# chrischoy/DeepGlobalRegistration

Measured on NVIDIA H100. Metric: scan_pairs_per_sec, higher is better.
Workload: dtype f32

## Files before the change

### deepglobalregistration_b200/_abi.py

```python
import ctypes as C
import math
import os
import re

import numpy as np
import torch

from .build import INCLUDE

_HERE = os.path.dirname(os.path.abspath(__file__))
LIB_PATH = os.path.join(_HERE, 'libdgr_b200.so')
HEADER = os.path.join(INCLUDE, 'dgr_b200.h')


class DgrError(RuntimeError):
  pass


_SCALARS = {'int32_t': C.c_int32, 'int64_t': C.c_int64, 'uint64_t': C.c_uint64, 'float': C.c_float,
            'double': C.c_double}


def _ctype(decl, c_type, ret=False):
  words = c_type.replace('*', ' * ').split()
# ... 252 lines not shown
  call('dgr_hash_find', ptr(coords), coords.shape[0], coords.shape[1], ptr(spec), ptr(table.keys),
       ptr(table.vals), table.cap, ptr(rows), stream())
  return rows


def gather_rows_i32(src, idx, n):
  out = torch.empty(n, src.shape[1], dtype=torch.int32, device=src.device)
  call('dgr_gather_rows_i32', ptr(src), ptr(idx), n, src.shape[1], ptr(out), stream())
  return out


def coarse_maps(fine, spec, strides):
  _chk(fine, torch.int32, 'fine')
  n, ncols = fine.shape
  L, nmx, dev = len(strides), max(n, 1), fine.device
  cap = table_cap(n)
  keys = torch.empty(L, cap, dtype=torch.int64, device=dev)
  vals = torch.empty(L, cap, dtype=torch.int32, device=dev)
  coords = torch.empty(L, nmx, ncols, dtype=torch.int32, device=dev)
  n_out = torch.empty(L, dtype=torch.int32, device=dev)
  slot = scratch('cm_slot', L * nmx, torch.int32, dev)
  scan = scratch('cm_scan', L * lib().dgr_scan_ws_elems(nmx), torch.int32, dev)
  call('dgr_coarse_maps', ptr(fine), n, None, ncols, ptr(spec), L, (C.c_int32 * L)(*strides), ptr(keys), ptr(vals),
       cap, ptr(coords), ptr(n_out), ptr(slot), ptr(scan), stream())
  return coords, [HashTable.wrap(keys[l], vals[l], cap) for l in range(L)], n_out


class KernelMap:
  __slots__ = ('K', 'n_in', 'n_out', 'nbr', 'in_idx', 'out_idx', 'kofs', 'kofs_host', 'n_pairs',
               'tile_k', 'tile_start', 'n_tiles', '_paired')

  def paired_tiles(self):
    if getattr(self, '_paired', None) is None:
      counts = self.kofs_host[1:] - self.kofs_host[:-1]
      per_k = (counts + TILE_ROWS - 1) // TILE_ROWS
      n = int(((per_k + 1) // 2 * 2).sum())
      dev = self.kofs.device
      tk = torch.empty(max(n, 1), dtype=torch.int32, device=dev)
      ts = torch.empty(max(n, 1), dtype=torch.int32, device=dev)
      call('dgr_kernel_map_tiles', ptr(self.kofs), self.K, TILE_ROWS, n, 1, ptr(tk), ptr(ts), stream())
      self._paired = (tk, ts, n)
    return self._paired

  def transposed(self):
    t = KernelMap()
    for k in self.__slots__:
      setattr(t, k, getattr(self, k, None))
    t.in_idx, t.out_idx = self.out_idx, self.in_idx
    t.n_in, t.n_out = self.n_out, self.n_in
    t.nbr = None
    return t


def kernel_map(out_coords, spec, in_table, n_in, offsets, keep_table=False):
  global D2H_BYTES
  _chk(out_coords, torch.int32, 'out_coords')
  _chk(offsets, torch.int32, 'offsets')
  dev = out_coords.device
  n_out, ncols = out_coords.shape
  K = offsets.shape[0]
  nmx = max(n_out, 1)
  bits = scratch('km_bits', K * lib().dgr_kmap_mask_words(nmx), torch.int32, dev)
  cnt = scratch('km_cnt', lib().dgr_kmap_cnt_elems(K, nmx), torch.int32, dev)
  kofs = torch.empty(K + 2, dtype=torch.int32, device=dev)
  meta = scratch('km_meta', 5, torch.int32, dev)
  bloom, n_words = None, 0
  if K > 27:
    n_words = lib().dgr_bloom2_words(n_in)
    bloom = scratch('km_bloom', n_words, torch.int32, dev)
    call('dgr_bloom2_build', ptr(in_table.keys), in_table.cap, ptr(bloom), n_words, stream())
  table = (ptr(in_table.keys), ptr(in_table.vals), in_table.cap)
  call('dgr_kmap_probe', ptr(out_coords), n_out, None, ncols, ptr(spec), *table, ptr(bloom), n_words, ptr(offsets), K,
       ptr(bits), ptr(cnt), ptr(kofs), ptr(meta), stream())
  km = KernelMap()
  km.nbr = None
  if keep_table:
    km.nbr = torch.empty(K, nmx, dtype=torch.int32, device=dev)
    call('dgr_kmap_dense', ptr(out_coords), n_out, None, ncols, ptr(spec), *table, ptr(bloom), n_words, ptr(offsets),
         K, ptr(km.nbr), nmx, None, stream())
  kofs_all = kofs.cpu().numpy()
  D2H_BYTES += kofs_all.nbytes
  if kofs_all[K + 1] != 0:
    raise DgrError('coordinate extent does not fit a 63-bit packed key')
  kofs_host = kofs_all[:K + 1]
  P = int(kofs_host[K])
  counts = kofs_host[1:] - kofs_host[:-1]
  n_tiles = int(((counts + TILE_ROWS - 1) // TILE_ROWS).sum())
  km.K, km.n_in, km.n_out = K, n_in, n_out
  km.in_idx = torch.empty(max(P, 1), dtype=torch.int32, device=dev)
  km.out_idx = torch.empty(max(P, 1), dtype=torch.int32, device=dev)
  km.tile_k = torch.empty(max(n_tiles, 1), dtype=torch.int32, device=dev)
  km.tile_start = torch.empty(max(n_tiles, 1), dtype=torch.int32, device=dev)
  if P > 0:
    call('dgr_kmap_fill', ptr(bits), ptr(cnt), K, n_out, ptr(out_coords), ncols, ptr(spec), *table, ptr(offsets),
         ptr(km.in_idx), ptr(km.out_idx), stream())
    call('dgr_kernel_map_tiles', ptr(kofs), K, TILE_ROWS, n_tiles, 0, ptr(km.tile_k), ptr(km.tile_start), stream())
  km.kofs, km.kofs_host, km.n_pairs, km.n_tiles = kofs, kofs_host, P, n_tiles
  km._paired = None
  return km


def spconv_fwd(feat, weight, km, out, relu_in=False):
  _chk(feat, torch.float32, 'feat'); _chk(weight, torch.float32, 'weight'); _chk(out, torch.float32, 'out')
  cin, cout = feat.shape[1], out.shape[1]
  assert weight.numel() == km.K * cin * cout, (weight.shape, km.K, cin, cout)
  assert feat.shape[0] == km.n_in and out.shape[0] == km.n_out, (feat.shape, out.shape, km.n_in, km.n_out)
  _conv_profiled('spconv_fwd_kernel', km, cin, cout, lambda: call(
      'dgr_spconv_fwd', ptr(feat), cin, ptr(weight), cout, ptr(km.in_idx), ptr(km.out_idx), ptr(km.kofs),
      ptr(km.tile_k), ptr(km.tile_start), km.n_tiles, TILE_ROWS, int(relu_in), ptr(out), stream()))
  return out


def spconv_wgrad(feat, grad_out, km):
  _chk(feat, torch.float32, 'feat'); _chk(grad_out, torch.float32, 'grad_out')
  cin, cout = feat.shape[1], grad_out.shape[1]
  dw = torch.empty(km.K, cin, cout, dtype=torch.float32, device=feat.device)
  call('dgr_spconv_wgrad', ptr(feat), cin, ptr(grad_out), cout, ptr(km.in_idx), ptr(km.out_idx), ptr(km.kofs), km.K,
       ptr(dw), stream())
  return dw


def tc_supported(cin, cout):
  return bool(lib().dgr_spconv_tc_supported(int(cin), int(cout)))


# ... 656 lines not shown
```

### deepglobalregistration_b200/csrc/coordplan.cu

```cuda
#include "common.cuh"

namespace {

constexpr int kThreads = 256;
constexpr int kCntWords = 256;
constexpr int kProbeThreads = 512;

template <typename T0, typename T1>
__global__ void compact_voxels_kernel(const int32_t* __restrict__ raw, const int32_t* __restrict__ sel,
                                      const int32_t* __restrict__ n_unique, int64_t n_raw0,
                                      const T0* __restrict__ xyz0, const T1* __restrict__ xyz1, double cell,
                                      int32_t* __restrict__ coords, float* __restrict__ xyz,
                                      int32_t* __restrict__ counts) {
  const int n = n_unique[0];
  if (blockIdx.x == 0 && threadIdx.x == 0) {
    int lo = 0, hi = n;
    while (lo < hi) {
      const int mid = (lo + hi) >> 1;
      if (sel[mid] < n_raw0) lo = mid + 1; else hi = mid;
    }
    counts[0] = n;
    counts[1] = lo;
    counts[2] = n - lo;
    counts[3] = n_unique[1];
  }
  for (int64_t i = (int64_t)blockIdx.x * blockDim.x + threadIdx.x; i < n; i += (int64_t)gridDim.x * blockDim.x) {
    const int64_t r = sel[i];
    const int4 k = reinterpret_cast<const int4*>(raw)[r];
    reinterpret_cast<int4*>(coords)[i] = k;
    double x, y, z;
    if (r < n_raw0) {
      x = (double)xyz0[3 * r]; y = (double)xyz0[3 * r + 1]; z = (double)xyz0[3 * r + 2];
    } else {
      const int64_t q = r - n_raw0;
      x = (double)xyz1[3 * q]; y = (double)xyz1[3 * q + 1]; z = (double)xyz1[3 * q + 2];
    }
    xyz[3 * i] = dgr_float32_in_cell(x, k.y, cell);
    xyz[3 * i + 1] = dgr_float32_in_cell(y, k.z, cell);
    xyz[3 * i + 2] = dgr_float32_in_cell(z, k.w, cell);
  }
}

__device__ __forceinline__ uint32_t bloom_mix(uint64_t key) {
  uint32_t h = (uint32_t)key ^ ((uint32_t)(key >> 32) * 0x9E3779B1u);
  h ^= h >> 16;
  h *= 0x85EBCA6Bu;
  h ^= h >> 13;
  h *= 0xC2B2AE35u;
  h ^= h >> 16;
  return h;
}
__device__ __forceinline__ uint32_t bloom_bits(uint32_t h) { return (1u << ((h >> 20) & 31)) | (1u << ((h >> 26) & 31)); }

__global__ void bloom2_build_kernel(const uint64_t* __restrict__ keys, int64_t cap, uint32_t* words,
                                    uint32_t word_mask) {
  int64_t i = (int64_t)blockIdx.x * blockDim.x + threadIdx.x;
  if (i >= cap) return;
  const uint64_t k = keys[i];
  if (k == DGR_EMPTY_KEY) return;
  const uint32_t h = bloom_mix(k);
  atomicOr(words + (h & word_mask), bloom_bits(h));
}

template <bool kBloom, bool kDense>
__global__ void __launch_bounds__(kProbeThreads, 2)
kmap_probe_kernel(const int32_t* __restrict__ out_coords, const int32_t* __restrict__ n_out_dev, int64_t n_out_max,
                  int ncols, const dgr_keyspec_t* __restrict__ spec_p, const uint64_t* __restrict__ keys,
                  const int32_t* __restrict__ vals, uint64_t mask, const uint32_t* __restrict__ bloom,
                  uint32_t n_bloom_words, const int32_t* __restrict__ offsets, int K, int k_per_block,
                  uint32_t* __restrict__ bits, int W, int32_t* block_cnt, int bpk, int32_t* __restrict__ nbr,
                  int64_t nbr_stride, int32_t* hit_count) {
  extern __shared__ __align__(16) unsigned char smem_raw[];
  constexpr int kWarps = kProbeThreads / 32;
  long long* delta = reinterpret_cast<long long*>(smem_raw);
  uint32_t* mtile = reinterpret_cast<uint32_t*>(smem_raw + (size_t)k_per_block * 8);
  uint16_t* queue = reinterpret_cast<uint16_t*>(mtile + (size_t)kWarps * k_per_block);
  uint32_t* bloom_s = reinterpret_cast<uint32_t*>(queue + kWarps * 64);
  const int n_out = dgr_dev_count(n_out_dev, n_out_max);
  const int k0 = blockIdx.y * k_per_block;
  const int kn = min(k_per_block, K - k0);
  const int lane = threadIdx.x & 31, warp = threadIdx.x >> 5;
  if ((int64_t)blockIdx.x * kProbeThreads >= n_out) {
    if (!kDense) {
      const int w = blockIdx.x * kWarps + warp;
      if (lane == 0 && w < W)
        for (int kk = 0; kk < kn; ++kk) bits[(int64_t)(k0 + kk) * W + w] = 0u;
    }
    return;
  }
  const dgr_keyspec_t s = *spec_p;
  for (int kk = threadIdx.x; kk < kn; kk += blockDim.x) {
    long long d = 0;
    const int32_t* o = offsets + (int64_t)(k0 + kk) * (ncols - 1);
    for (int a = 0; a < ncols - 1; ++a) d += (long long)o[a] * (1ll << s.shift[a + 1]);
    delta[kk] = d;
  }
  if (!kDense)
    for (int e = threadIdx.x; e < kWarps * k_per_block; e += blockDim.x) mtile[e] = 0u;
  if (kBloom)
    for (uint32_t i = threadIdx.x; i < n_bloom_words; i += blockDim.x) bloom_s[i] = bloom[i];
  __syncthreads();
  const int64_t j = (int64_t)blockIdx.x * kProbeThreads + threadIdx.x;
  const bool live = j < n_out;
  const uint64_t key = live ? dgr_pack_key(out_coords + j * ncols, s) : 0;
  const uint32_t key_lo = (uint32_t)key, key_hi = (uint32_t)(key >> 32);
  const int64_t row0 = j - lane;
  const uint32_t wm = n_bloom_words - 1;
  uint16_t* q = queue + warp * 64;
  uint32_t* mt = mtile + warp * k_per_block;
  int qn = 0;

  auto drain = [&](int count) {
    __syncwarp();
    const uint32_t e = lane < count ? q[lane] : 0u;
    const int src = e & 31, kq = e >> 5;
    const uint32_t lo = __shfl_sync(0xffffffffu, key_lo, src), hi = __shfl_sync(0xffffffffu, key_hi, src);
    if (lane < count) {
      const uint64_t qq = (((uint64_t)hi << 32) | lo) + (uint64_t)delta[kq];
      const int32_t i = dgr_hash_lookup(keys, vals, mask, qq);
      if (kDense) {
        nbr[(int64_t)(k0 + kq) * nbr_stride + row0 + src] = i;
        if (hit_count != nullptr) {
          const uint32_t act = __activemask();
          const uint32_t hits = __ballot_sync(act, i >= 0);
          if (lane == (__ffs(act) - 1) && hits) atomicAdd(hit_count, __popc(hits));
        }
      } else if (i >= 0) {
        atomicOr(mt + kq, 1u << src);
      }
    }
    __syncwarp();
    const uint32_t rest = (lane + 32 < qn) ? q[lane + 32] : 0u;
    __syncwarp();
    if (lane + 32 < qn) q[lane] = (uint16_t)rest;
    qn = qn > 32 ? qn - 32 : 0;
    __syncwarp();
  };

  if (!kBloom && !kDense) {
    const int w = (int)(j >> 5);
    const int cnt_col = w / kCntWords;
    for (int kk = 0; kk < kn; kk += 4) {
      bool found[4];
#pragma unroll
      for (int u = 0; u < 4; ++u)
        found[u] = live && kk + u < kn && dgr_hash_lookup(keys, vals, mask, key + (uint64_t)delta[min(kk + u, kn - 1)]) >= 0;
#pragma unroll
      for (int u = 0; u < 4; ++u) {
        if (kk + u >= kn) break;
        const uint32_t m = __ballot_sync(0xffffffffu, found[u]);
        if (lane == 0 && w < W) {
          bits[(int64_t)(k0 + kk + u) * W + w] = m;
          if (m) atomicAdd(block_cnt + (int64_t)(k0 + kk + u) * bpk + cnt_col, __popc(m));
        }
      }
    }
    return;
  }
  for (int kk = 0; kk < kn; ++kk) {
    bool maybe = live;
    if (kBloom && live) {
      const uint32_t h = bloom_mix(key + (uint64_t)delta[kk]);
      const uint32_t b = bloom_bits(h);
      maybe = (bloom_s[h & wm] & b) == b;
    }
    if (kDense && live && !maybe) nbr[(int64_t)(k0 + kk) * nbr_stride + j] = -1;
    const uint32_t cand = __ballot_sync(0xffffffffu, maybe);
    if (cand) {
      if (maybe) q[qn + __popc(cand & ((1u << lane) - 1u))] = (uint16_t)((kk << 5) | lane);
      qn += __popc(cand);
      if (qn >= 32) drain(32);
    }
  }
  if (qn > 0) drain(qn);
  if (!kDense) {
    __syncwarp();
    const int w = (int)(j >> 5);
    if (w < W) {
      const int cnt_col = w / kCntWords;
      for (int kk = lane; kk < kn; kk += 32) {
        const uint32_t m = mt[kk];
        bits[(int64_t)(k0 + kk) * W + w] = m;
        if (m) atomicAdd(block_cnt + (int64_t)(k0 + kk) * bpk + cnt_col, __popc(m));
      }
    }
  }
}

__global__ void kmap_scan_kernel(int32_t* cnt, int K, int bpk, int tile_rows, int32_t* kofs,
                                 int32_t* meta, const dgr_keyspec_t* spec) {
  const int64_t nb = (int64_t)K * bpk;
  const int total = dgr_block_scan_inplace(cnt, nb);
  if (threadIdx.x == 0) cnt[nb] = total;
  __syncthreads();
  __shared__ int red[3][32];
  int tiles = 0, ptiles = 0, nonempty = 0;
  for (int k = threadIdx.x; k <= K; k += blockDim.x) {
    const int lo = cnt[(int64_t)k * bpk];
    kofs[k] = lo;
    if (k < K) {
      const int hi = (k + 1 < K) ? cnt[(int64_t)(k + 1) * bpk] : total;
      const int t = (hi - lo + tile_rows - 1) / tile_rows;
      tiles += t;
      ptiles += (t + 1) & ~1;
      nonempty += (hi > lo);
    }
  }
#pragma unroll
  for (int d = 16; d > 0; d >>= 1) {
    tiles += __shfl_xor_sync(0xffffffffu, tiles, d);
    ptiles += __shfl_xor_sync(0xffffffffu, ptiles, d);
    nonempty += __shfl_xor_sync(0xffffffffu, nonempty, d);
  }
  if ((threadIdx.x & 31) == 0) {
    red[0][threadIdx.x >> 5] = tiles;
    red[1][threadIdx.x >> 5] = ptiles;
    red[2][threadIdx.x >> 5] = nonempty;
  }
  __syncthreads();
  if (threadIdx.x == 0) {
    int a = 0, b = 0, c = 0;
    for (int w = 0; w < (int)(blockDim.x >> 5); ++w) { a += red[0][w]; b += red[1][w]; c += red[2][w]; }
    const int ovf = spec != nullptr ? spec->overflow : 0;
    kofs[K + 1] = ovf;
    meta[0] = total; meta[1] = a; meta[2] = b; meta[3] = c; meta[4] = ovf;
  }
}

__global__ void __launch_bounds__(kThreads)
kmap_fill_kernel(const uint32_t* __restrict__ bits, int W, int bpk, const int32_t* __restrict__ block_ofs,
                 const int32_t* __restrict__ out_coords, int ncols, const dgr_keyspec_t* __restrict__ spec_p,
                 const uint64_t* __restrict__ keys, const int32_t* __restrict__ vals, uint64_t mask,
                 const int32_t* __restrict__ offsets, int32_t* __restrict__ in_idx, int32_t* __restrict__ out_idx) {
  __shared__ uint32_t s_mask[kThreads];
  __shared__ int s_base[kThreads];
  const int kappa = blockIdx.y;
  const int64_t e = (int64_t)kappa * bpk + blockIdx.x;
  const int base = block_ofs[e];
  if (block_ofs[e + 1] == base) return;
// ... 57 lines not shown
  const int64_t n_max = n_raw0 + n_raw1;
  unsigned blocks = dgr_blocks(n_max > 0 ? n_max : 1, kThreads);
  if (blocks > 1184) blocks = 1184;
#define DGR_CV(T0, T1)                                                                                         \
  compact_voxels_kernel<T0, T1><<<blocks, kThreads, 0, st>>>(raw_coords, sel, n_unique, n_raw0, (const T0*)xyz0, \
                                                             (const T1*)xyz1, cell, coords, xyz, counts)
  if (is_f64_0 && is_f64_1) DGR_CV(double, double);
  else if (is_f64_0) DGR_CV(double, float);
  else if (is_f64_1) DGR_CV(float, double);
  else DGR_CV(float, float);
#undef DGR_CV
  dgr_note_launches(1);
  DGR_LAUNCH_CHECK();
  return DGR_OK;
}

int32_t dgr_bloom2_build(const uint64_t* keys, int64_t cap, uint32_t* words, int64_t n_words, void* stream) {
  DGR_ARG_CHECK(cap > 0 && (cap & (cap - 1)) == 0, "capacity must be a power of two");
  DGR_ARG_CHECK(n_words >= 32 && (n_words & (n_words - 1)) == 0, "n_words must be a power of two");
  cudaStream_t st = (cudaStream_t)stream;
  DGR_CUDA_CHECK(cudaMemsetAsync(words, 0, (size_t)n_words * 4, st));
  bloom2_build_kernel<<<dgr_blocks(cap, kThreads), kThreads, 0, st>>>(keys, cap, words, (uint32_t)n_words - 1);
  dgr_note_launches(1);
  DGR_LAUNCH_CHECK();
  return DGR_OK;
}

int64_t dgr_bloom2_words(int64_t n_max) {
  int64_t words = 1;
  while (words < (n_max * 10 + 31) / 32) words <<= 1;
  return words < 1024 ? 1024 : (words > 16384 ? 16384 : words);
}

int64_t dgr_kmap_mask_words(int64_t n_out_max) {
  const int64_t w = (n_out_max + 31) / 32;
  return w < 1 ? 1 : w;
}
int64_t dgr_kmap_cnt_elems(int32_t K, int64_t n_out_max) {
  const int64_t W = dgr_kmap_mask_words(n_out_max);
  return (int64_t)K * ((W + kCntWords - 1) / kCntWords) + 2;
}

static size_t probe_smem_bytes(int k_per_block, int64_t n_bloom_words) {
  return (size_t)k_per_block * 8 + (size_t)(kProbeThreads / 32) * k_per_block * 4 + (size_t)(kProbeThreads / 32) * 64 * 2 +
         (size_t)n_bloom_words * 4;
}
static int probe_k_per_block(int K, unsigned row_blocks) {
  int k_per_block = K;
  while (k_per_block > 16 && (int64_t)row_blocks * ((K + k_per_block - 1) / k_per_block) < 528) k_per_block = (k_per_block + 1) / 2;
  if (k_per_block > 96) k_per_block = 96;
  return (k_per_block + 3) & ~3;
}

int32_t dgr_kmap_probe(const int32_t* out_coords, int64_t n_out_max, const int32_t* n_out_dev, int32_t ncols,
                       const dgr_keyspec_t* spec, const uint64_t* in_keys, const int32_t* in_vals, int64_t in_cap,
                       const uint32_t* bloom_words, int64_t n_bloom_words, const int32_t* offsets, int32_t K,
                       uint32_t* bits, int32_t* block_cnt, int32_t* kofs, int32_t* meta, void* stream) {
  DGR_ARG_CHECK(in_cap > 0 && (in_cap & (in_cap - 1)) == 0, "capacity must be a power of two");
  DGR_ARG_CHECK(K >= 1 && K <= 65535, "K out of range");
  DGR_ARG_CHECK(bloom_words == nullptr || (n_bloom_words >= 32 && (n_bloom_words & (n_bloom_words - 1)) == 0 &&
                                           n_bloom_words <= 32768),
                "bloom: power of two, 32..32768 words");
  cudaStream_t st = (cudaStream_t)stream;
  const int64_t nmx = n_out_max > 0 ? n_out_max : 1;
  const int W = (int)dgr_kmap_mask_words(nmx);
  const int bpk = (W + kCntWords - 1) / kCntWords;
  DGR_CUDA_CHECK(cudaMemsetAsync(block_cnt, 0, (size_t)dgr_kmap_cnt_elems(K, nmx) * sizeof(int32_t), st));
  const unsigned row_blocks = dgr_blocks(nmx, kProbeThreads);
  const int k_per_block = probe_k_per_block(K, row_blocks);
  const dim3 grid(row_blocks, (K + k_per_block - 1) / k_per_block);
  if (bloom_words != nullptr) {
    const size_t smem = probe_smem_bytes(k_per_block, n_bloom_words);
    DGR_ENSURE_SMEM((kmap_probe_kernel<true, false>), smem);
    kmap_probe_kernel<true, false><<<grid, kProbeThreads, smem, st>>>(
        out_coords, n_out_dev, n_out_max, ncols, spec, in_keys, in_vals, (uint64_t)in_cap - 1, bloom_words,
        (uint32_t)n_bloom_words, offsets, K, k_per_block, bits, W, block_cnt, bpk, nullptr, 0, nullptr);
  } else {
    const size_t smem = probe_smem_bytes(k_per_block, 0);
    kmap_probe_kernel<false, false><<<grid, kProbeThreads, smem, st>>>(
        out_coords, n_out_dev, n_out_max, ncols, spec, in_keys, in_vals, (uint64_t)in_cap - 1, nullptr, 1u, offsets, K,
        k_per_block, bits, W, block_cnt, bpk, nullptr, 0, nullptr);
  }
  kmap_scan_kernel<<<1, 1024, 0, st>>>(block_cnt, K, bpk, 128, kofs, meta, spec);
  dgr_note_launches(2);
  DGR_LAUNCH_CHECK();
  return DGR_OK;
}

int32_t dgr_kmap_fill(const uint32_t* bits, const int32_t* block_cnt, int32_t K, int64_t n_out_max,
                      const int32_t* out_coords, int32_t ncols, const dgr_keyspec_t* spec,
                      const uint64_t* in_keys, const int32_t* in_vals, int64_t in_cap, const int32_t* offsets,
                      int32_t* in_idx, int32_t* out_idx, void* stream) {
  const int64_t nmx = n_out_max > 0 ? n_out_max : 1;
  const int W = (int)dgr_kmap_mask_words(nmx);
  const int bpk = (W + kCntWords - 1) / kCntWords;
  kmap_fill_kernel<<<dim3(bpk, K), kThreads, 0, (cudaStream_t)stream>>>(bits, W, bpk, block_cnt, out_coords, ncols,
                                                                            spec, in_keys, in_vals, (uint64_t)in_cap - 1,
                                                                            offsets, in_idx, out_idx);
  dgr_note_launches(1);
  DGR_LAUNCH_CHECK();
  return DGR_OK;
}

int32_t dgr_kmap_dense(const int32_t* out_coords, int64_t n_out_max, const int32_t* n_out_dev, int32_t ncols,
                       const dgr_keyspec_t* spec, const uint64_t* in_keys, const int32_t* in_vals, int64_t in_cap,
                       const uint32_t* bloom_words, int64_t n_bloom_words, const int32_t* offsets, int32_t K,
                       int32_t* nbr, int64_t nbr_stride, int32_t* hit_count, void* stream) {
  DGR_ARG_CHECK(in_cap > 0 && (in_cap & (in_cap - 1)) == 0, "capacity must be a power of two");
  DGR_ARG_CHECK(nbr_stride >= n_out_max, "row stride below the row bound");
  if (hit_count != nullptr) DGR_CUDA_CHECK(cudaMemsetAsync(hit_count, 0, sizeof(int32_t), (cudaStream_t)stream));
  DGR_ARG_CHECK(bloom_words == nullptr || (n_bloom_words >= 32 && (n_bloom_words & (n_bloom_words - 1)) == 0 &&
                                           n_bloom_words <= 32768),
                "bloom: power of two, 32..32768 words");
  if (n_out_max == 0) return DGR_OK;
  cudaStream_t st = (cudaStream_t)stream;
  const unsigned row_blocks = dgr_blocks(n_out_max, kProbeThreads);
  const int k_per_block = probe_k_per_block(K, row_blocks);
  const dim3 grid(row_blocks, (K + k_per_block - 1) / k_per_block);
  if (bloom_words != nullptr) {
    const size_t smem = probe_smem_bytes(k_per_block, n_bloom_words);
    DGR_ENSURE_SMEM((kmap_probe_kernel<true, true>), smem);
    kmap_probe_kernel<true, true><<<grid, kProbeThreads, smem, st>>>(
        out_coords, n_out_dev, n_out_max, ncols, spec, in_keys, in_vals, (uint64_t)in_cap - 1, bloom_words,
        (uint32_t)n_bloom_words, offsets, K, k_per_block, nullptr, 0, nullptr, 0, nbr, nbr_stride, hit_count);
  } else {
    const size_t smem = probe_smem_bytes(k_per_block, 0);
    kmap_probe_kernel<false, true><<<grid, kProbeThreads, smem, st>>>(
        out_coords, n_out_dev, n_out_max, ncols, spec, in_keys, in_vals, (uint64_t)in_cap - 1, nullptr, 1u, offsets, K,
        k_per_block, nullptr, 0, nullptr, 0, nbr, nbr_stride, hit_count);
  }
  dgr_note_launches(1);
  DGR_LAUNCH_CHECK();
  return DGR_OK;
}

int32_t dgr_kernel_map_tiles(const int32_t* kofs, int32_t K, int32_t tile_rows, int32_t n_tiles, int32_t pair,
                             int32_t* tile_k, int32_t* tile_start, void* stream) {
  DGR_ARG_CHECK(tile_rows >= 1, "tile_rows must be positive");
  if (n_tiles == 0) return DGR_OK;
  tiles_kernel<<<1, 1024, (K + 1) * sizeof(int), (cudaStream_t)stream>>>(kofs, K, tile_rows, n_tiles, pair, tile_k,
                                                                        tile_start);
  dgr_note_launches(1);
  DGR_LAUNCH_CHECK();
  return DGR_OK;
}

}
```

### deepglobalregistration_b200/csrc/exec.cu

```cuda
#include <math.h>
#include <stdlib.h>
#include <string.h>

#include <map>
#include <tuple>
#include <vector>

#include <nvtx3/nvToolsExt.h>

#include "common.cuh"

namespace {

constexpr int kTileRows = 128;
constexpr int kMetaInts = 256;
constexpr int kMetaNetBase = 8;
constexpr int kMetaPerMap = 5;
constexpr int kKeyMargin = 32;

bool tc_f16_enabled();
int tc_f16_min_cout();

__global__ void fill_f32_kernel(float* p, int64_t n, float v) {
  int64_t i = (int64_t)blockIdx.x * blockDim.x + threadIdx.x;
// ... 293 lines not shown
    L.n_max = n_max;
    L.n_dev = n_out_dev + (l - 1);
    L.keys = keys + (int64_t)(l - 1) * cap;
    L.vals = vals + (int64_t)(l - 1) * cap;
    L.cap = cap;
  }
  const bool use_bloom = p.D > 3;
  if (use_bloom || net->conv1_ks > 3) {
    const int64_t words = dgr_bloom2_words(n_max);
    for (int l = 0; l < (use_bloom ? 4 : 1); ++l) {
      DGR_TRY(aalloc(c, words, &p.lv[l].bloom));
      p.lv[l].n_bloom = words;
      DGR_TRY(dgr_bloom2_build(p.lv[l].keys, p.lv[l].cap, p.lv[l].bloom, words, st));
    }
  }
  p.n_maps = 0;
  auto add_map = [&](int lin, int lout, int ksize, bool dense) {
    KMap& m = p.maps[p.n_maps];
    m = KMap();
    m.lin = lin; m.lout = lout; m.ksize = ksize; m.dense = dense;
    m.K = 1;
    for (int a = 0; a < p.D; ++a) m.K *= ksize;
    return p.n_maps++;
  };
  for (int l = 0; l < 4; ++l) p.map_same[l] = add_map(l, l, 3, false);
  for (int l = 0; l < 3; ++l) p.map_down[l] = add_map(l, l + 1, 3, false);
  if (net->conv1_ks == 3) {
    p.map_conv1 = p.map_same[0];
  } else {
    const bool bits_only = conv1_table_kernel(net) && p.input_ones && net->in_ch == 1;
    p.map_conv1 = add_map(0, 0, net->conv1_ks, conv1_table_kernel(net) && !bits_only);
    p.maps[p.map_conv1].bits_only = bits_only;
  }
  for (int i = 0; i < p.n_maps; ++i) {
    KMap& m = p.maps[i];
    const Level& Lin = p.lv[m.lin];
    const Level& Lout = p.lv[m.lout];
    DGR_TRY(get_offsets(c, m.ksize, p.D, 1 << m.lin, &m.offsets));
    m.meta = c->meta_dev + p.meta_base + 4 + kMetaPerMap * i;
    if (m.dense) {
      m.nbr_stride = nmx;
      DGR_TRY(aalloc(c, (int64_t)m.K * nmx, &m.nbr));
      const bool bloom = Lin.bloom != nullptr && m.K > 27;
      DGR_CUDA_CHECK(cudaMemsetAsync(m.meta, 0, kMetaPerMap * sizeof(int32_t), (cudaStream_t)st));
      DGR_TRY(dgr_kmap_dense(Lout.coords, Lout.n_max, Lout.n_dev, ncols, p.spec, Lin.keys, Lin.vals, Lin.cap,
                             bloom ? Lin.bloom : nullptr, bloom ? Lin.n_bloom : 0, m.offsets, m.K, m.nbr, m.nbr_stride,
                             m.meta, st));
      continue;
    }
    m.W = dgr_kmap_mask_words(nmx);
    DGR_TRY(aalloc(c, (int64_t)m.K * m.W, &m.bits));
    DGR_TRY(aalloc(c, dgr_kmap_cnt_elems(m.K, nmx), &m.cnt));
    DGR_TRY(aalloc(c, m.K + 2, &m.kofs));
    const bool bloom = Lin.bloom != nullptr && m.K > 27;
    DGR_TRY(dgr_kmap_probe(Lout.coords, Lout.n_max, Lout.n_dev, ncols, p.spec, Lin.keys, Lin.vals, Lin.cap,
                           bloom ? Lin.bloom : nullptr, bloom ? Lin.n_bloom : 0, m.offsets, m.K, m.bits, m.cnt, m.kofs,
                           m.meta, st));
  }
  return DGR_OK;
}

int32_t plan_finish(dgr_ctx* c, Plan& p) {
  void* st = c->stream;
  const int32_t* mh = c->meta_host + p.meta_base;
  for (int l = 1; l < 4; ++l) p.lv[l].n = mh[l];
  for (int i = 0; i < p.n_maps; ++i) {
    KMap& m = p.maps[i];
    const int32_t* mm = mh + 4 + kMetaPerMap * i;
    if (m.dense || m.bits_only) {
      m.P = mm[0];
      m.nonempty = m.dense ? m.K : mm[3];
      continue;
    }
    m.P = mm[0]; m.n_tiles = mm[1]; m.nonempty = mm[3];
    if (mm[4] != 0) {
      dgr_set_error("coordinate extent does not fit a 63-bit packed key");
      return DGR_ERR_ARG;
    }
    const Level& Lin = p.lv[m.lin];
    const Level& Lout = p.lv[m.lout];
    DGR_TRY(aalloc(c, m.P, &m.in_idx));
    DGR_TRY(aalloc(c, m.P, &m.out_idx));
    DGR_TRY(aalloc(c, m.n_tiles, &m.tile_k));
    DGR_TRY(aalloc(c, m.n_tiles, &m.tile_start));
    if (m.P > 0) {
      DGR_TRY(dgr_kmap_fill(m.bits, m.cnt, m.K, Lout.n_max > 0 ? Lout.n_max : 1, Lout.coords, p.ncols, p.spec, Lin.keys,
                            Lin.vals, Lin.cap, m.offsets, m.in_idx, m.out_idx, st));
      DGR_TRY(dgr_kernel_map_tiles(m.kofs, m.K, kTileRows, m.n_tiles, 0, m.tile_k, m.tile_start, st));
    }
  }
  return DGR_OK;
}

struct LayerExec {
  const Conv* conv;
  const KMap* map;
  bool transposed;
  int n_in, n_out;
  bool table;
  bool bits;
};

bool tc_f16_enabled() {
  static const bool v = [] {
    const char* e = getenv("DGR_TC_F16");
    return e ? atoi(e) != 0 : true;
  }();
  return v;
}
int tc_f16_min_cout() {
// ... 600 lines not shown
```

### deepglobalregistration_b200/me/coords.py

```python
import numpy as np
import torch

from .. import _abi
from .._abi import KEY_MARGIN


class CoordinateMapKey:
  __slots__ = ('stride', 'tag')

  def __init__(self, stride, tag=''):
    self.stride, self.tag = int(stride), tag

  def get_tensor_stride(self):
    return self.stride

  def __eq__(self, o):
    return isinstance(o, CoordinateMapKey) and (self.stride, self.tag) == (o.stride, o.tag)

  def __hash__(self):
    return hash((self.stride, self.tag))

  def __repr__(self):
    return f'CoordinateMapKey(stride={self.stride})'

# ... 30 lines not shown
      spec = _abi.keyspec_build(_abi.coords_minmax(coords), coords.shape[1], KEY_MARGIN)
      table, _, _, cnt = _abi.unique_first(coords, spec)
      n_unique = _abi.read_count(cnt)
      if n_unique != coords.shape[0]:
        raise ValueError(f'{coords.shape[0] - n_unique} duplicate coordinates: the DGR hot path feeds '
                         'unique coordinates (sparse_quantize output) and relies on row order')
    coords = coords.detach()
    self.device = coords.device
    self.D = coords.shape[1] - 1
    self.spec = spec
    self._maps = {1: _Map(coords, table, coords.shape[0])}
    self._kmaps = {}
    self._offsets = {}

  @staticmethod
  def _check_spec(spec):
    if int(spec[1].item()) != 0:
      raise _abi.DgrError('coordinate extent does not fit a 63-bit packed key')

  def origin_key(self):
    return CoordinateMapKey(1)

  def num_rows(self, key):
    return self._map(key.stride).n

  def coordinates(self, key):
    return self._map(key.stride).coords

  def _map(self, stride):
    if stride not in self._maps:
      assert stride % 2 == 0 and stride > 1, f'no coordinate map at stride {stride}'
      coords, tables, n_out = _abi.coarse_maps(self._maps[1].coords, self.spec, [stride])
      n, overflow = torch.cat([n_out, self.spec[1:2]]).cpu().tolist()
      _abi.D2H_BYTES += 8
      if overflow:
        raise _abi.DgrError('coordinate extent does not fit a 63-bit packed key')
      self._maps[stride] = _Map(coords[0, :n], tables[0], n)
    return self._maps[stride]

  def _offs(self, kernel_size, stride):
    k = (kernel_size, self.D, stride, self.device)
    if k not in _OFFSET_CACHE:
      _OFFSET_CACHE[k] = kernel_offsets(kernel_size, self.D, stride, self.device)
    return _OFFSET_CACHE[k]

  def kernel_map(self, in_key, conv_stride, kernel_size):
    s_in = in_key.stride
    s_out = s_in * conv_stride
    ck = (s_in, s_out, kernel_size)
    if ck not in self._kmaps:
      m_in, m_out = self._map(s_in), self._map(s_out)
      keep = self.D == 3 and conv_stride == 1 and kernel_size > 3
      self._kmaps[ck] = _abi.kernel_map(m_out.coords, self.spec, m_in.table, m_in.n,
                                        self._offs(kernel_size, s_in), keep_table=keep)
    return CoordinateMapKey(s_out), self._kmaps[ck]

  def transpose_kernel_map(self, in_key, conv_stride, kernel_size):
    s_in = in_key.stride
    assert s_in % conv_stride == 0, 'transposed convolution below tensor stride 1'
    s_out = s_in // conv_stride
    if conv_stride == 1:
      return self.kernel_map(in_key, 1, kernel_size)
    ck = (s_out, s_in, kernel_size)
    if ck not in self._kmaps:
      raise NotImplementedError('transposed convolution without a matching strided convolution '
                                '(generating new coordinates) is not on the DGR hot path')
    tk = ('T',) + ck
    if tk not in self._kmaps:
      self._kmaps[tk] = self._kmaps[ck].transposed()
    return CoordinateMapKey(s_out), self._kmaps[tk]
```

### include/dgr_b200.h

```cpp
#ifndef DGR_B200_H_
#define DGR_B200_H_

#include <stdint.h>

#ifdef __cplusplus
extern "C" {
#endif

#define DGR_OK 0
#define DGR_ERR_CUDA (-1)
#define DGR_ERR_ARG (-2)
#define DGR_ERR_DEVICE (-3)

#define DGR_MAX_COLS 8

typedef struct dgr_keyspec {
  int32_t ncols;
  int32_t overflow;
  int32_t lo[DGR_MAX_COLS];
  int32_t shift[DGR_MAX_COLS];
  int32_t bits[DGR_MAX_COLS];
} dgr_keyspec_t;

int32_t dgr_version(void);
// ... 211 lines not shown
                      int32_t* base_log, double* result, void* stream);

#define DGR_POINTNET_PARAMS 154368
#define DGR_POINTNET_PACKED_BYTES 1185792
int32_t dgr_pointnet_pack(const double* params, void* packed, void* stream);
int32_t dgr_pointnet_forward(const float* points, int64_t n, const double* centre, const double* poses, int32_t n_poses,
                             const void* packed, float* features, void* stream);
int32_t dgr_pointnetlk_ws_elems(int64_t n_src, int64_t n_tgt, int32_t max_iter, int64_t* n_elems);
int32_t dgr_pointnetlk(const float* src, int64_t n_src, const float* tgt, int64_t n_tgt, const void* packed,
                       double delta, int32_t max_iter, double xtol, uint64_t* ws, double* jac_out, double* log,
                       double* result, void* stream);


int32_t dgr_spconv_table_fwd_strided(const float* in_feat, int32_t cin, const float* weight, int32_t cout,
                                     const int32_t* nbr, int32_t K, int64_t n_out, int64_t nbr_stride,
                                     const float* scale, const float* shift, float* out, void* stream);

int32_t dgr_spconv_wgrad(const float* in_feat, int32_t cin, const float* grad_out, int32_t cout,
                         const int32_t* in_idx, const int32_t* out_idx, const int32_t* kofs, int32_t K, float* dw,
                         void* stream);

int32_t dgr_affine_act_amax(const float* x, int64_t n, int32_t c, const float* scale, const float* shift,
                            const float* residual, int32_t relu, float* out, float* amax, void* stream);
int32_t dgr_absmax_f32(const float* x, int64_t n, float* amax, void* stream);
int32_t dgr_spconv_tc_f16_supported(int32_t cin, int32_t cout);
int32_t dgr_pack_weight_f16(const float* w, int32_t K, int32_t cin, int32_t cout, void* packed, float* scale_ws,
                            void* stream);
int32_t dgr_spconv_tc_f16_fwd(const float* in_feat, int32_t cin, const void* weight_h, int32_t cout,
                              const int32_t* in_idx, const int32_t* out_idx, const int32_t* kofs,
                              const int32_t* tile_k, const int32_t* tile_start, int32_t n_tiles, int32_t tile_rows,
                              const float* amax_in, const float* w_scale, float* out, void* stream);

int32_t dgr_spconv_ones_bits_fwd(const float* weight, int32_t cout, const uint32_t* bits, int64_t mask_words, int32_t K,
                                 int64_t n_out, const float* scale, const float* shift, float* out, void* stream);

int32_t dgr_compact_voxel_pair(const int32_t* raw_coords, const int32_t* sel, const int32_t* n_unique,
                               int64_t n_raw0, int64_t n_raw1, const void* xyz0, int32_t is_f64_0, const void* xyz1,
                               int32_t is_f64_1, double cell, int32_t* coords, float* xyz, int32_t* counts,
                               void* stream);
int32_t dgr_table_build_unique(const int32_t* coords, int64_t n_max, const int32_t* n_dev, int32_t ncols,
                               const dgr_keyspec_t* spec, uint64_t* keys, int32_t* vals, int64_t cap, void* stream);
int32_t dgr_coarse_maps(const int32_t* fine, int64_t n_max, const int32_t* n_dev, int32_t ncols,
                        const dgr_keyspec_t* spec, int32_t n_levels, const int32_t* strides, uint64_t* keys,
                        int32_t* vals, int64_t cap, int32_t* coords_out, int32_t* n_out, int32_t* slot_ws,
                        int32_t* scan_ws, void* stream);
int32_t dgr_bloom2_build(const uint64_t* keys, int64_t cap, uint32_t* words, int64_t n_words, void* stream);
int64_t dgr_bloom2_words(int64_t n_max);
int64_t dgr_kmap_mask_words(int64_t n_out_max);
int64_t dgr_kmap_cnt_elems(int32_t K, int64_t n_out_max);
int32_t dgr_kmap_probe(const int32_t* out_coords, int64_t n_out_max, const int32_t* n_out_dev, int32_t ncols,
                       const dgr_keyspec_t* spec, const uint64_t* in_keys, const int32_t* in_vals, int64_t in_cap,
                       const uint32_t* bloom_words, int64_t n_bloom_words, const int32_t* offsets, int32_t K,
                       uint32_t* bits, int32_t* block_cnt, int32_t* kofs, int32_t* meta, void* stream);
int32_t dgr_kmap_fill(const uint32_t* bits, const int32_t* block_cnt, int32_t K, int64_t n_out_max,
                      const int32_t* out_coords, int32_t ncols, const dgr_keyspec_t* spec, const uint64_t* in_keys,
                      const int32_t* in_vals, int64_t in_cap, const int32_t* offsets, int32_t* in_idx,
                      int32_t* out_idx, void* stream);
int32_t dgr_kernel_map_tiles(const int32_t* kofs, int32_t K, int32_t tile_rows, int32_t n_tiles, int32_t pair,
                             int32_t* tile_k, int32_t* tile_start, void* stream);
int32_t dgr_kmap_dense(const int32_t* out_coords, int64_t n_out_max, const int32_t* n_out_dev, int32_t ncols,
                       const dgr_keyspec_t* spec, const uint64_t* in_keys, const int32_t* in_vals, int64_t in_cap,
                       const uint32_t* bloom_words, int64_t n_bloom_words, const int32_t* offsets, int32_t K,
                       int32_t* nbr, int64_t nbr_stride, int32_t* hit_count, void* stream);

typedef struct dgr_ctx dgr_ctx_t;
typedef struct dgr_net dgr_net_t;
int32_t dgr_ctx_create(int32_t device, void* stream , dgr_ctx_t** out);
int32_t dgr_ctx_destroy(dgr_ctx_t* ctx);
void* dgr_ctx_stream(dgr_ctx_t* ctx);
int32_t dgr_ctx_stats(dgr_ctx_t* ctx, int64_t* stats);
int32_t dgr_ctx_profile(dgr_ctx_t* ctx, int32_t enable);
int64_t dgr_ctx_profile_read(dgr_ctx_t* ctx, double* rows, int64_t max_rows);
int32_t dgr_ctx_stage_times(dgr_ctx_t* ctx, double* ms, int32_t max_stages);

int32_t dgr_net_create(int32_t device, int32_t D, int32_t in_ch, int32_t out_ch, int32_t conv1_ks, int32_t normalize,
                       const int32_t* channels, const int32_t* tr_channels, const float* const* params,
                       int32_t n_params, void* stream, dgr_net_t** out);
int32_t dgr_net_destroy(dgr_net_t* net);
int32_t dgr_net_forward(dgr_ctx_t* ctx, dgr_net_t* net, const int32_t* coords, int64_t n, const float* feats,
                        float* out);

int32_t dgr_pair_register(dgr_ctx_t* ctx, dgr_net_t* fcgf, dgr_net_t* inlier, const void* xyz0, int64_t n_raw0,
                          int32_t is_f64_0, const void* xyz1, int64_t n_raw1, int32_t is_f64_1, int32_t on_host,
                          double voxel, float clip, int32_t use_icp, double* result);
int32_t dgr_pair_safeguard(dgr_ctx_t* ctx, double max_dist, int64_t num_hyp, uint64_t seed, int32_t use_icp,
                           double* result);
int32_t dgr_pair_tap(dgr_ctx_t* ctx, int32_t which, int64_t* rows, int32_t* cols, void* dst);

#ifdef __cplusplus
}
#endif
#endif
```

Measured before the change: 80.84.

## Exploit kernel-map symmetry for same-stride and invert probing for stride-2 downsampling

For same-stride convolutions with an odd centred kernel, only half of the offsets are probed in the hash table. Each hit is mirrored into the opposite offset's bitmask with atomicOr, and the centre offset is filled from the live mask. For stride-2 kernel-3 downsampling, each input point instead enumerates only the output cells that can contain it and looks them up in the output table. A separate count kernel then fills the per-block counts for offsets that were set by atomics. This is meant to cut hash lookups roughly in half or more during kernel-map construction, at the cost of scattered global atomics, extra memsets and one extra launch.

```diff
diff --git a/deepglobalregistration_b200/_abi.py b/deepglobalregistration_b200/_abi.py
--- a/deepglobalregistration_b200/_abi.py
+++ b/deepglobalregistration_b200/_abi.py
@@ -328,7 +328,20 @@
     return t
 
 
-def kernel_map(out_coords, spec, in_table, n_in, offsets, keep_table=False):
+KMAP_GENERAL, KMAP_SAME, KMAP_DOWN = (_DEFINES['DGR_KMAP_GENERAL'], _DEFINES['DGR_KMAP_SAME'],
+                                     _DEFINES['DGR_KMAP_DOWN'])
+
+
+def kmap_mode(s_in, s_out, kernel_size):
+  if s_out == s_in and kernel_size % 2 == 1 and kernel_size > 1:
+    return KMAP_SAME
+  if s_out == 2 * s_in and kernel_size == 3:
+    return KMAP_DOWN
+  return KMAP_GENERAL
+
+
+def kernel_map(out_coords, spec, in_table, n_in, offsets, keep_table=False, mode=KMAP_GENERAL, in_coords=None,
+               in_stride=0, out_table=None):
   global D2H_BYTES
   _chk(out_coords, torch.int32, 'out_coords')
   _chk(offsets, torch.int32, 'offsets')
@@ -341,12 +354,15 @@
   kofs = torch.empty(K + 2, dtype=torch.int32, device=dev)
   meta = scratch('km_meta', 5, torch.int32, dev)
   bloom, n_words = None, 0
-  if K > 27:
+  if K > 27 and mode != KMAP_DOWN:
     n_words = lib().dgr_bloom2_words(n_in)
     bloom = scratch('km_bloom', n_words, torch.int32, dev)
     call('dgr_bloom2_build', ptr(in_table.keys), in_table.cap, ptr(bloom), n_words, stream())
   table = (ptr(in_table.keys), ptr(in_table.vals), in_table.cap)
-  call('dgr_kmap_probe', ptr(out_coords), n_out, None, ncols, ptr(spec), *table, ptr(bloom), n_words, ptr(offsets), K,
+  down = mode == KMAP_DOWN
+  call('dgr_kmap_probe_mode', mode, ptr(out_coords), n_out, None, ncols, ptr(spec), *table, ptr(bloom), n_words,
+       ptr(offsets), K, ptr(in_coords) if down else None, n_in if down else 0, None, in_stride if down else 0,
+       ptr(out_table.keys) if down else None, ptr(out_table.vals) if down else None, out_table.cap if down else 0,
        ptr(bits), ptr(cnt), ptr(kofs), ptr(meta), stream())
   km = KernelMap()
   km.nbr = None
diff --git a/deepglobalregistration_b200/csrc/coordplan.cu b/deepglobalregistration_b200/csrc/coordplan.cu
--- a/deepglobalregistration_b200/csrc/coordplan.cu
+++ b/deepglobalregistration_b200/csrc/coordplan.cu
@@ -62,14 +62,14 @@
   atomicOr(words + (h & word_mask), bloom_bits(h));
 }
 
-template <bool kBloom, bool kDense>
+template <bool kBloom, bool kDense, bool kSym>
 __global__ void __launch_bounds__(kProbeThreads, 2)
 kmap_probe_kernel(const int32_t* __restrict__ out_coords, const int32_t* __restrict__ n_out_dev, int64_t n_out_max,
                   int ncols, const dgr_keyspec_t* __restrict__ spec_p, const uint64_t* __restrict__ keys,
                   const int32_t* __restrict__ vals, uint64_t mask, const uint32_t* __restrict__ bloom,
                   uint32_t n_bloom_words, const int32_t* __restrict__ offsets, int K, int k_per_block,
                   uint32_t* __restrict__ bits, int W, int32_t* block_cnt, int bpk, int32_t* __restrict__ nbr,
-                  int64_t nbr_stride, int32_t* hit_count) {
+                  int64_t nbr_stride, int32_t* hit_count, int k_last) {
   extern __shared__ __align__(16) unsigned char smem_raw[];
   constexpr int kWarps = kProbeThreads / 32;
   long long* delta = reinterpret_cast<long long*>(smem_raw);
@@ -109,6 +109,13 @@
   uint16_t* q = queue + warp * 64;
   uint32_t* mt = mtile + warp * k_per_block;
   int qn = 0;
+  auto mirror = [&](int kappa, int32_t i) {
+    atomicOr(bits + (int64_t)(k_last - kappa) * W + (i >> 5), 1u << (i & 31));
+  };
+  if (kSym && blockIdx.y == 0) {
+    const uint32_t m = __ballot_sync(0xffffffffu, live);
+    if (lane == 0 && (j >> 5) < W) bits[(int64_t)(k_last / 2) * W + (j >> 5)] = m;
+  }
 
   auto drain = [&](int count) {
     __syncwarp();
@@ -127,6 +134,7 @@
         }
       } else if (i >= 0) {
         atomicOr(mt + kq, 1u << src);
+        if (kSym) mirror(k0 + kq, i);
       }
     }
     __syncwarp();
@@ -141,14 +149,15 @@
     const int w = (int)(j >> 5);
     const int cnt_col = w / kCntWords;
     for (int kk = 0; kk < kn; kk += 4) {
-      bool found[4];
+      int32_t found[4];
 #pragma unroll
       for (int u = 0; u < 4; ++u)
-        found[u] = live && kk + u < kn && dgr_hash_lookup(keys, vals, mask, key + (uint64_t)delta[min(kk + u, kn - 1)]) >= 0;
+        found[u] = live && kk + u < kn ? dgr_hash_lookup(keys, vals, mask, key + (uint64_t)delta[min(kk + u, kn - 1)]) : -1;
 #pragma unroll
       for (int u = 0; u < 4; ++u) {
         if (kk + u >= kn) break;
-        const uint32_t m = __ballot_sync(0xffffffffu, found[u]);
+        if (kSym && found[u] >= 0) mirror(k0 + kk + u, found[u]);
+        const uint32_t m = __ballot_sync(0xffffffffu, found[u] >= 0);
         if (lane == 0 && w < W) {
           bits[(int64_t)(k0 + kk + u) * W + w] = m;
           if (m) atomicAdd(block_cnt + (int64_t)(k0 + kk + u) * bpk + cnt_col, __popc(m));
@@ -185,6 +194,53 @@
       }
     }
   }
+}
+
+constexpr int kDownLanes = 8;
+__global__ void __launch_bounds__(kThreads)
+kmap_down_kernel(const int32_t* __restrict__ in_coords, const int32_t* __restrict__ n_in_dev, int64_t n_in_max,
+                 int ncols, int stride, const dgr_keyspec_t* __restrict__ spec_p, const uint64_t* __restrict__ out_keys,
+                 const int32_t* __restrict__ out_vals, uint64_t out_mask, uint32_t* __restrict__ bits, int W) {
+  const int n_in = dgr_dev_count(n_in_dev, n_in_max);
+  const int64_t t = (int64_t)blockIdx.x * blockDim.x + threadIdx.x;
+  const int64_t i = t / kDownLanes;
+  if (i >= n_in) return;
+  const dgr_keyspec_t s = *spec_p;
+  const int32_t* c = in_coords + i * ncols;
+  const uint64_t key = dgr_pack_key(c, s);
+  uint32_t odd = 0;
+#pragma unroll
+  for (int a = 1; a < DGR_MAX_COLS; ++a)
+    if (a < ncols) odd |= (uint32_t)((c[a] / stride) & 1) << a;
+  const uint32_t n_cand = 1u << __popc(odd);
+  for (uint32_t sub = (uint32_t)(t % kDownLanes); sub < n_cand; sub += kDownLanes) {
+    int kappa = 0, p = 1, b = 0;
+    long long d = 0;
+#pragma unroll
+    for (int a = 1; a < DGR_MAX_COLS; ++a) {
+      if (a < ncols) {
+        int digit = 1;
+        if ((odd >> a) & 1u) {
+          const long long step = (long long)stride << s.shift[a];
+          if ((sub >> b++) & 1u) { digit = 2; d -= step; }
+          else { digit = 0; d += step; }
+        }
+        kappa += digit * p;
+        p *= 3;
+      }
+    }
+    const int32_t o = dgr_hash_lookup(out_keys, out_vals, out_mask, key + (uint64_t)d);
+    if (o >= 0) atomicOr(bits + (int64_t)kappa * W + (o >> 5), 1u << (o & 31));
+  }
+}
+
+__global__ void __launch_bounds__(kThreads)
+kmap_count_kernel(const uint32_t* __restrict__ bits, int W, int bpk, int k_lo, int32_t* __restrict__ block_cnt) {
+  const int64_t kappa = k_lo + blockIdx.y;
+  const int w = blockIdx.x * kCntWords + threadIdx.x;
+  int total;
+  dgr_block_exclusive_scan<kThreads>(w < W ? __popc(bits[kappa * W + w]) : 0, &total);
+  if (threadIdx.x == 0) block_cnt[kappa * bpk + blockIdx.x] = total;
 }
 
 __global__ void kmap_scan_kernel(int32_t* cnt, int K, int bpk, int tile_rows, int32_t* kofs,
@@ -348,39 +404,78 @@
   return (k_per_block + 3) & ~3;
 }
 
-int32_t dgr_kmap_probe(const int32_t* out_coords, int64_t n_out_max, const int32_t* n_out_dev, int32_t ncols,
-                       const dgr_keyspec_t* spec, const uint64_t* in_keys, const int32_t* in_vals, int64_t in_cap,
-                       const uint32_t* bloom_words, int64_t n_bloom_words, const int32_t* offsets, int32_t K,
-                       uint32_t* bits, int32_t* block_cnt, int32_t* kofs, int32_t* meta, void* stream) {
+int32_t dgr_kmap_probe_mode(int32_t mode, const int32_t* out_coords, int64_t n_out_max, const int32_t* n_out_dev,
+                            int32_t ncols, const dgr_keyspec_t* spec, const uint64_t* in_keys, const int32_t* in_vals,
+                            int64_t in_cap, const uint32_t* bloom_words, int64_t n_bloom_words, const int32_t* offsets,
+                            int32_t K, const int32_t* in_coords, int64_t n_in_max, const int32_t* n_in_dev,
+                            int32_t in_stride, const uint64_t* out_keys, const int32_t* out_vals, int64_t out_cap,
+                            uint32_t* bits, int32_t* block_cnt, int32_t* kofs, int32_t* meta, void* stream) {
+  DGR_ARG_CHECK(mode == DGR_KMAP_GENERAL || mode == DGR_KMAP_SAME || mode == DGR_KMAP_DOWN, "unknown probe mode");
   DGR_ARG_CHECK(in_cap > 0 && (in_cap & (in_cap - 1)) == 0, "capacity must be a power of two");
   DGR_ARG_CHECK(K >= 1 && K <= 65535, "K out of range");
   DGR_ARG_CHECK(bloom_words == nullptr || (n_bloom_words >= 32 && (n_bloom_words & (n_bloom_words - 1)) == 0 &&
                                            n_bloom_words <= 32768),
                 "bloom: power of two, 32..32768 words");
+  DGR_ARG_CHECK(mode != DGR_KMAP_SAME || (K > 1 && (K & 1)), "same-stride mode: a centred odd cube of offsets");
+  if (mode == DGR_KMAP_DOWN) {
+    int64_t k3 = 1;
+    for (int a = 1; a < ncols; ++a) k3 *= 3;
+    DGR_ARG_CHECK(K == k3, "down mode: kernel size 3");
+    DGR_ARG_CHECK(in_coords != nullptr && in_stride >= 1 && n_in_max >= 0, "down mode: input rows and stride");
+    DGR_ARG_CHECK(out_keys != nullptr && out_vals != nullptr && out_cap > 0 && (out_cap & (out_cap - 1)) == 0,
+                  "down mode: output table, capacity a power of two");
+  }
   cudaStream_t st = (cudaStream_t)stream;
   const int64_t nmx = n_out_max > 0 ? n_out_max : 1;
   const int W = (int)dgr_kmap_mask_words(nmx);
   const int bpk = (W + kCntWords - 1) / kCntWords;
   DGR_CUDA_CHECK(cudaMemsetAsync(block_cnt, 0, (size_t)dgr_kmap_cnt_elems(K, nmx) * sizeof(int32_t), st));
-  const unsigned row_blocks = dgr_blocks(nmx, kProbeThreads);
-  const int k_per_block = probe_k_per_block(K, row_blocks);
-  const dim3 grid(row_blocks, (K + k_per_block - 1) / k_per_block);
-  if (bloom_words != nullptr) {
-    const size_t smem = probe_smem_bytes(k_per_block, n_bloom_words);
-    DGR_ENSURE_SMEM((kmap_probe_kernel<true, false>), smem);
-    kmap_probe_kernel<true, false><<<grid, kProbeThreads, smem, st>>>(
-        out_coords, n_out_dev, n_out_max, ncols, spec, in_keys, in_vals, (uint64_t)in_cap - 1, bloom_words,
-        (uint32_t)n_bloom_words, offsets, K, k_per_block, bits, W, block_cnt, bpk, nullptr, 0, nullptr);
+  int k_counted = K;
+  if (mode == DGR_KMAP_DOWN) {
+    DGR_CUDA_CHECK(cudaMemsetAsync(bits, 0, (size_t)K * W * sizeof(uint32_t), st));
+    if (n_in_max > 0)
+      kmap_down_kernel<<<dgr_blocks(n_in_max * kDownLanes, kThreads), kThreads, 0, st>>>(
+          in_coords, n_in_dev, n_in_max, ncols, in_stride, spec, out_keys, out_vals, (uint64_t)out_cap - 1, bits, W);
+    k_counted = 0;
   } else {
-    const size_t smem = probe_smem_bytes(k_per_block, 0);
-    kmap_probe_kernel<false, false><<<grid, kProbeThreads, smem, st>>>(
-        out_coords, n_out_dev, n_out_max, ncols, spec, in_keys, in_vals, (uint64_t)in_cap - 1, nullptr, 1u, offsets, K,
-        k_per_block, bits, W, block_cnt, bpk, nullptr, 0, nullptr);
-  }
+    const bool sym = mode == DGR_KMAP_SAME;
+    const int Kp = sym ? (K - 1) / 2 : K;
+    if (sym) DGR_CUDA_CHECK(cudaMemsetAsync(bits + (int64_t)Kp * W, 0, (size_t)(K - Kp) * W * sizeof(uint32_t), st));
+    k_counted = Kp;
+    const unsigned row_blocks = dgr_blocks(nmx, kProbeThreads);
+    const int k_per_block = probe_k_per_block(Kp, row_blocks);
+    const dim3 grid(row_blocks, (Kp + k_per_block - 1) / k_per_block);
+    const uint32_t* bw = bloom_words;
+    const uint32_t nbw = bloom_words != nullptr ? (uint32_t)n_bloom_words : 1u;
+    const size_t smem = probe_smem_bytes(k_per_block, bloom_words != nullptr ? n_bloom_words : 0);
+#define DGR_PROBE(B, S)                                                                                             \
+  do {                                                                                                              \
+    DGR_ENSURE_SMEM((kmap_probe_kernel<B, false, S>), smem);                                                       \
+    kmap_probe_kernel<B, false, S><<<grid, kProbeThreads, smem, st>>>(                                              \
+        out_coords, n_out_dev, n_out_max, ncols, spec, in_keys, in_vals, (uint64_t)in_cap - 1, bw, nbw, offsets, Kp, \
+        k_per_block, bits, W, block_cnt, bpk, nullptr, 0, nullptr, K - 1);                                          \
+  } while (0)
+    if (bloom_words != nullptr) {
+      if (sym) DGR_PROBE(true, true); else DGR_PROBE(true, false);
+    } else {
+      if (sym) DGR_PROBE(false, true); else DGR_PROBE(false, false);
+    }
+#undef DGR_PROBE
+  }
+  if (k_counted < K) kmap_count_kernel<<<dim3(bpk, K - k_counted), kThreads, 0, st>>>(bits, W, bpk, k_counted, block_cnt);
   kmap_scan_kernel<<<1, 1024, 0, st>>>(block_cnt, K, bpk, 128, kofs, meta, spec);
-  dgr_note_launches(2);
+  dgr_note_launches(k_counted < K ? 3 : 2);
   DGR_LAUNCH_CHECK();
   return DGR_OK;
+}
+
+int32_t dgr_kmap_probe(const int32_t* out_coords, int64_t n_out_max, const int32_t* n_out_dev, int32_t ncols,
+                       const dgr_keyspec_t* spec, const uint64_t* in_keys, const int32_t* in_vals, int64_t in_cap,
+                       const uint32_t* bloom_words, int64_t n_bloom_words, const int32_t* offsets, int32_t K,
+                       uint32_t* bits, int32_t* block_cnt, int32_t* kofs, int32_t* meta, void* stream) {
+  return dgr_kmap_probe_mode(DGR_KMAP_GENERAL, out_coords, n_out_max, n_out_dev, ncols, spec, in_keys, in_vals, in_cap,
+                             bloom_words, n_bloom_words, offsets, K, nullptr, 0, nullptr, 0, nullptr, nullptr, 0, bits,
+                             block_cnt, kofs, meta, stream);
 }
 
 int32_t dgr_kmap_fill(const uint32_t* bits, const int32_t* block_cnt, int32_t K, int64_t n_out_max,
@@ -415,15 +510,15 @@
   const dim3 grid(row_blocks, (K + k_per_block - 1) / k_per_block);
   if (bloom_words != nullptr) {
     const size_t smem = probe_smem_bytes(k_per_block, n_bloom_words);
-    DGR_ENSURE_SMEM((kmap_probe_kernel<true, true>), smem);
-    kmap_probe_kernel<true, true><<<grid, kProbeThreads, smem, st>>>(
+    DGR_ENSURE_SMEM((kmap_probe_kernel<true, true, false>), smem);
+    kmap_probe_kernel<true, true, false><<<grid, kProbeThreads, smem, st>>>(
         out_coords, n_out_dev, n_out_max, ncols, spec, in_keys, in_vals, (uint64_t)in_cap - 1, bloom_words,
-        (uint32_t)n_bloom_words, offsets, K, k_per_block, nullptr, 0, nullptr, 0, nbr, nbr_stride, hit_count);
+        (uint32_t)n_bloom_words, offsets, K, k_per_block, nullptr, 0, nullptr, 0, nbr, nbr_stride, hit_count, 0);
   } else {
     const size_t smem = probe_smem_bytes(k_per_block, 0);
-    kmap_probe_kernel<false, true><<<grid, kProbeThreads, smem, st>>>(
+    kmap_probe_kernel<false, true, false><<<grid, kProbeThreads, smem, st>>>(
         out_coords, n_out_dev, n_out_max, ncols, spec, in_keys, in_vals, (uint64_t)in_cap - 1, nullptr, 1u, offsets, K,
-        k_per_block, nullptr, 0, nullptr, 0, nbr, nbr_stride, hit_count);
+        k_per_block, nullptr, 0, nullptr, 0, nbr, nbr_stride, hit_count, 0);
   }
   dgr_note_launches(1);
   DGR_LAUNCH_CHECK();
diff --git a/deepglobalregistration_b200/csrc/exec.cu b/deepglobalregistration_b200/csrc/exec.cu
--- a/deepglobalregistration_b200/csrc/exec.cu
+++ b/deepglobalregistration_b200/csrc/exec.cu
@@ -369,10 +369,14 @@
     DGR_TRY(aalloc(c, (int64_t)m.K * m.W, &m.bits));
     DGR_TRY(aalloc(c, dgr_kmap_cnt_elems(m.K, nmx), &m.cnt));
     DGR_TRY(aalloc(c, m.K + 2, &m.kofs));
-    const bool bloom = Lin.bloom != nullptr && m.K > 27;
-    DGR_TRY(dgr_kmap_probe(Lout.coords, Lout.n_max, Lout.n_dev, ncols, p.spec, Lin.keys, Lin.vals, Lin.cap,
-                           bloom ? Lin.bloom : nullptr, bloom ? Lin.n_bloom : 0, m.offsets, m.K, m.bits, m.cnt, m.kofs,
-                           m.meta, st));
+    const bool down = m.lout == m.lin + 1 && m.ksize == 3;
+    const int mode = m.lout == m.lin ? DGR_KMAP_SAME : (down ? DGR_KMAP_DOWN : DGR_KMAP_GENERAL);
+    const bool bloom = Lin.bloom != nullptr && m.K > 27 && !down;
+    DGR_TRY(dgr_kmap_probe_mode(mode, Lout.coords, Lout.n_max, Lout.n_dev, ncols, p.spec, Lin.keys, Lin.vals, Lin.cap,
+                                bloom ? Lin.bloom : nullptr, bloom ? Lin.n_bloom : 0, m.offsets, m.K,
+                                down ? Lin.coords : nullptr, down ? Lin.n_max : 0, down ? Lin.n_dev : nullptr,
+                                down ? 1 << m.lin : 0, down ? Lout.keys : nullptr, down ? Lout.vals : nullptr,
+                                down ? Lout.cap : 0, m.bits, m.cnt, m.kofs, m.meta, st));
   }
   return DGR_OK;
 }
diff --git a/deepglobalregistration_b200/me/coords.py b/deepglobalregistration_b200/me/coords.py
--- a/deepglobalregistration_b200/me/coords.py
+++ b/deepglobalregistration_b200/me/coords.py
@@ -106,7 +106,9 @@
       m_in, m_out = self._map(s_in), self._map(s_out)
       keep = self.D == 3 and conv_stride == 1 and kernel_size > 3
       self._kmaps[ck] = _abi.kernel_map(m_out.coords, self.spec, m_in.table, m_in.n,
-                                        self._offs(kernel_size, s_in), keep_table=keep)
+                                        self._offs(kernel_size, s_in), keep_table=keep,
+                                        mode=_abi.kmap_mode(s_in, s_out, kernel_size), in_coords=m_in.coords,
+                                        in_stride=s_in, out_table=m_out.table)
     return CoordinateMapKey(s_out), self._kmaps[ck]
 
   def transpose_kernel_map(self, in_key, conv_stride, kernel_size):
diff --git a/include/dgr_b200.h b/include/dgr_b200.h
--- a/include/dgr_b200.h
+++ b/include/dgr_b200.h
@@ -287,6 +287,15 @@
                        const dgr_keyspec_t* spec, const uint64_t* in_keys, const int32_t* in_vals, int64_t in_cap,
                        const uint32_t* bloom_words, int64_t n_bloom_words, const int32_t* offsets, int32_t K,
                        uint32_t* bits, int32_t* block_cnt, int32_t* kofs, int32_t* meta, void* stream);
+#define DGR_KMAP_GENERAL 0
+#define DGR_KMAP_SAME 1
+#define DGR_KMAP_DOWN 2
+int32_t dgr_kmap_probe_mode(int32_t mode, const int32_t* out_coords, int64_t n_out_max, const int32_t* n_out_dev,
+                            int32_t ncols, const dgr_keyspec_t* spec, const uint64_t* in_keys, const int32_t* in_vals,
+                            int64_t in_cap, const uint32_t* bloom_words, int64_t n_bloom_words, const int32_t* offsets,
+                            int32_t K, const int32_t* in_coords, int64_t n_in_max, const int32_t* n_in_dev,
+                            int32_t in_stride, const uint64_t* out_keys, const int32_t* out_vals, int64_t out_cap,
+                            uint32_t* bits, int32_t* block_cnt, int32_t* kofs, int32_t* meta, void* stream);
 int32_t dgr_kmap_fill(const uint32_t* bits, const int32_t* block_cnt, int32_t K, int64_t n_out_max,
                       const int32_t* out_coords, int32_t ncols, const dgr_keyspec_t* spec, const uint64_t* in_keys,
                       const int32_t* in_vals, int64_t in_cap, const int32_t* offsets, int32_t* in_idx,
```

After: 84.66 (median of 6 runs). 4.7% higher.
